# bghira/SimpleTuner

Hardware: NVIDIA H100
Metric: images/sec Flux.1-dev LoRA bf16 1024^2 (higher is better)
Workload: dtype bf16

## Files before the change

simpletuner_b200/csrc/api.cu:

```cuda
#include <cuda.h>
#include <cudaTypedefs.h>
#include <cuda_runtime.h>

#include <algorithm>
#include <atomic>
#include <cstdarg>
#include <cstdio>
#include <cmath>
#include <cstdlib>
#include <cstring>
#include <mutex>
#include <string>
#include <unordered_map>

#include <climits>
#include "../../include/stb200.h"
#include "attn_bwd.cuh"
#include "attn_fwd.cuh"
#include "optim.cuh"
#include "elementwise.cuh"
#include "gemm.cuh"
#include "lokr.cuh"
#include "vae.cuh"
#include "wgrad.cuh"

namespace {

thread_local std::string g_err;
std::atomic<long long> g_launches{0};

int fail(int code, const char* fmt, ...) {
  char buf[512];
  va_list ap;
  va_start(ap, fmt);
  vsnprintf(buf, sizeof buf, fmt, ap);
  va_end(ap);
  g_err = buf;
  return code;
}

#define STB_CUDA(expr)                                                                       \
  do {                                                                                       \
    cudaError_t e_ = (expr);                                                                 \
    if (e_ != cudaSuccess) return fail(STB_ERR_CUDA, "%s: %s", #expr, cudaGetErrorString(e_)); \
  } while (0)

#define STB_LAUNCH_CHECK(name)                                                                  \
  do {                                                                                          \
    cudaError_t e_ = cudaGetLastError();                                                        \
    if (e_ != cudaSuccess) return fail(STB_ERR_CUDA, "launch %s: %s", name, cudaGetErrorString(e_)); \
    g_launches.fetch_add(1, std::memory_order_relaxed);                                         \
  } while (0)

int num_sms() {
  static int n = [] {
    int dev = 0, v = 0;
    if (cudaGetDevice(&dev) != cudaSuccess) return 0;
    if (cudaDeviceGetAttribute(&v, cudaDevAttrMultiProcessorCount, dev) != cudaSuccess) return 0;
    return v;
  }();
  return n;
}

int check_device() {
  static int ok = [] {
    int dev = 0, major = 0;
    if (cudaGetDevice(&dev) != cudaSuccess) return 0;
    if (cudaDeviceGetAttribute(&major, cudaDevAttrComputeCapabilityMajor, dev) != cudaSuccess) return 0;
    int minor = 0;
    if (cudaDeviceGetAttribute(&minor, cudaDevAttrComputeCapabilityMinor, dev) != cudaSuccess) return 0;
    return major == 9 && minor == 0 ? 1 : 0;
  }();
  if (!ok) return fail(STB_ERR_UNSUPPORTED, "libstb200 needs an sm_90 (H100) device; there is no CPU or other-arch fallback");
  return 0;
}

PFN_cuTensorMapEncodeTiled_v12000 encode_fn() {
  static PFN_cuTensorMapEncodeTiled_v12000 fn = [] {
    void* p = nullptr;
    cudaDriverEntryPointQueryResult q;
    if (cudaGetDriverEntryPoint("cuTensorMapEncodeTiled", &p, cudaEnableDefault, &q) != cudaSuccess) p = nullptr;
    return reinterpret_cast<PFN_cuTensorMapEncodeTiled_v12000>(p);
  }();
  return fn;
}

struct MapKey {
  const void* ptr;
  int rank;
  unsigned long long dims[4];
  unsigned long long strides[3];
  unsigned box[4];
  bool operator==(const MapKey& o) const { return std::memcmp(this, &o, sizeof(MapKey)) == 0; }
};
struct MapKeyHash {
  size_t operator()(const MapKey& k) const {
    const unsigned char* p = reinterpret_cast<const unsigned char*>(&k);
    size_t h = 1469598103934665603ull;
    for (size_t i = 0; i < sizeof(MapKey); ++i) h = (h ^ p[i]) * 1099511628211ull;
    return h;
  }
};
std::mutex g_map_mu;
std::unordered_map<MapKey, CUtensorMap, MapKeyHash> g_maps;

int make_map_strided(CUtensorMap* out, const void* ptr, int rank, const unsigned long long* dims,
                     const unsigned long long* strides_bytes, const unsigned* box, const unsigned* estrides) {
  auto fn = encode_fn();
  if (!fn) return fail(STB_ERR_CUDA, "cuTensorMapEncodeTiled entry point not available");
  if (reinterpret_cast<uintptr_t>(ptr) & 15) return fail(STB_ERR_ARG, "tensor base pointer must be 16-byte aligned");
  for (int i = 0; i + 1 < rank; ++i)
    if (strides_bytes[i] & 15) return fail(STB_ERR_ARG, "tensor stride %d (%llu bytes) must be a multiple of 16 bytes", i, strides_bytes[i]);
  cuuint64_t gdim[4];
  cuuint64_t gstr[3];
  cuuint32_t bx[4], es[4];
  for (int i = 0; i < rank; ++i) gdim[i] = dims[i], bx[i] = box[i], es[i] = estrides[i];
  for (int i = 0; i + 1 < rank; ++i) gstr[i] = strides_bytes[i];
  CUresult r = fn(out, CU_TENSOR_MAP_DATA_TYPE_BFLOAT16, rank, const_cast<void*>(ptr), gdim, gstr, bx, es,
                  CU_TENSOR_MAP_INTERLEAVE_NONE, CU_TENSOR_MAP_SWIZZLE_128B, CU_TENSOR_MAP_L2_PROMOTION_L2_256B,
                  CU_TENSOR_MAP_FLOAT_OOB_FILL_NONE);
  if (r != CUDA_SUCCESS) return fail(STB_ERR_CUDA, "cuTensorMapEncodeTiled failed with CUresult %d", int(r));
  return 0;
}

int make_map(CUtensorMap* out, const void* ptr, int rank, const unsigned long long* dims,
             const unsigned long long* strides_bytes, const unsigned* box) {
  MapKey key;
  std::memset(&key, 0, sizeof key);
  key.ptr = ptr;
  key.rank = rank;
  for (int i = 0; i < rank; ++i) key.dims[i] = dims[i], key.box[i] = box[i];
  for (int i = 0; i + 1 < rank; ++i) key.strides[i] = strides_bytes[i];
  {
    std::lock_guard<std::mutex> lk(g_map_mu);
    auto it = g_maps.find(key);
    if (it != g_maps.end()) {
      *out = it->second;
      return 0;
    }
  }
  static const unsigned unit[4] = {1, 1, 1, 1};
  if (int r = make_map_strided(out, ptr, rank, dims, strides_bytes, box, unit)) return r;
  {
    std::lock_guard<std::mutex> lk(g_map_mu);
    if (g_maps.size() > 65536) g_maps.clear();
    g_maps.emplace(key, *out);
  }
  return 0;
}

int make_token_map(CUtensorMap* out, const void* ptr, int C, int S, int B, long long s_stride, long long b_stride,
                   unsigned rows) {
  const unsigned long long d[3] = {(unsigned long long)C, (unsigned long long)S, (unsigned long long)B};
  const unsigned long long sb[2] = {(unsigned long long)s_stride * 2ull,
                                    (unsigned long long)(B == 1 ? s_stride * (long long)S : b_stride) * 2ull};
  const unsigned bx[3] = {64, rows, 1};
  return make_map(out, ptr, 3, d, sb, bx);
}

int make_head_map(CUtensorMap* out, const void* ptr, int HD, int H, int S, int B, long long sb, long long ss,
                  long long sh, unsigned rows) {
  const unsigned long long d[4] = {(unsigned long long)HD, (unsigned long long)H, (unsigned long long)S, (unsigned long long)B};
  const unsigned long long s[3] = {(unsigned long long)sh * 2ull, (unsigned long long)ss * 2ull, (unsigned long long)sb * 2ull};
  const unsigned bx[4] = {64, 1, rows, 1};
  return make_map(out, ptr, 4, d, s, bx);
}

template <auto Kernel>
int set_smem(int bytes) {
  static std::atomic<bool> done{false};
  if (done.load(std::memory_order_acquire)) return 0;
  STB_CUDA(cudaFuncSetAttribute(Kernel, cudaFuncAttributeMaxDynamicSharedMemorySize, bytes));
  done.store(true, std::memory_order_release);
  return 0;
}

template <int BN, int EPI, bool CONV>
int launch_gemm_kernel(const stb::GemmMaps& maps, const stb::GemmParams& p, cudaStream_t st, const char* name) {
  using Cfg = stb::GemmCfg<BN>;
  if (int r = set_smem<stb::gemm_bf16_tn_kernel<BN, EPI, CONV>>(Cfg::SMEM_BYTES)) return r;
  const long long tiles = (long long)((p.rows_per_batch + Cfg::BM - 1) / Cfg::BM) * p.num_batches * ((p.N + BN - 1) / BN);
  const int grid = (int)std::min<long long>(tiles, num_sms());
  stb::gemm_bf16_tn_kernel<BN, EPI, CONV><<<grid, 384, Cfg::SMEM_BYTES, st>>>(maps, p);
  STB_LAUNCH_CHECK(name);
  return 0;
}

template <int BN>
int launch_gemm(const stb_gemm_args* a, cudaStream_t st) {
  stb::GemmMaps maps;
  std::memset(&maps, 0, sizeof maps);
  stb::GemmParams p;
  std::memset(&p, 0, sizeof p);
  for (int s = 0; s < a->nseg; ++s) {
    const stb_gemm_seg& g = a->seg[s];
    if (g.K <= 0 || (g.K & 7)) return fail(STB_ERR_ARG, "segment %d: K=%d must be a positive multiple of 8", s, g.K);
    if (int r = make_token_map(&maps.a[s], g.a, g.K, a->rows_per_batch, a->num_batches, g.a_row_stride, g.a_batch_stride,
                               stb::GemmCfg<BN>::BM))
      return r;
    if (g.w_kn) {
      unsigned long long wd[2] = {(unsigned long long)a->N, (unsigned long long)g.K};
      unsigned long long ws[1] = {(unsigned long long)g.w_row_stride * 2ull};
      unsigned wb[2] = {64, 64};
      if (int r = make_map(&maps.w[s], g.w, 2, wd, ws, wb)) return r;
    } else {
      unsigned long long wd[2] = {(unsigned long long)g.K, (unsigned long long)a->N};
      unsigned long long ws[1] = {(unsigned long long)g.w_row_stride * 2ull};
      unsigned wb[2] = {64, (unsigned)BN};
      if (int r = make_map(&maps.w[s], g.w, 2, wd, ws, wb)) return r;
    }
    p.w_kn[s] = g.w_kn ? 1 : 0;
    p.kblocks[s] = (g.K + 63) / 64;
  }
  p.rows_per_batch = a->rows_per_batch;
  p.num_batches = a->num_batches;
  p.N = a->N;
  p.nseg = a->nseg;
  p.nan_to_num = a->nan_to_num;
  p.D = static_cast<__nv_bfloat16*>(a->d);
  p.d_batch_stride = a->d_batch_stride;
  p.d_row_stride = a->d_row_stride;
  p.bias = static_cast<const __nv_bfloat16*>(a->bias);
  p.gate = static_cast<const __nv_bfloat16*>(a->gate);
  p.gate_batch_stride = a->gate_batch_stride;
  p.res = static_cast<const __nv_bfloat16*>(a->res);
  p.res_batch_stride = a->res_batch_stride;
  p.res_row_stride = a->res_row_stride;
  p.aux = static_cast<__nv_bfloat16*>(a->aux);
  p.aux_batch_stride = a->aux_batch_stride;
  p.aux_row_stride = a->aux_row_stride;
  switch (a->epi) {
    case stb::EPI_STORE: return launch_gemm_kernel<BN, stb::EPI_STORE, false>(maps, p, st, "gemm_bf16_tn");
    case stb::EPI_GELU: return launch_gemm_kernel<BN, stb::EPI_GELU, false>(maps, p, st, "gemm_bf16_tn");
    case stb::EPI_GATE_RES: return launch_gemm_kernel<BN, stb::EPI_GATE_RES, false>(maps, p, st, "gemm_bf16_tn");
    case stb::EPI_MUL_DGELU: return launch_gemm_kernel<BN, stb::EPI_MUL_DGELU, false>(maps, p, st, "gemm_bf16_tn");
    case stb::EPI_ADD_RES: return launch_gemm_kernel<BN, stb::EPI_ADD_RES, false>(maps, p, st, "gemm_bf16_tn");
    case stb::EPI_MUL: return launch_gemm_kernel<BN, stb::EPI_MUL, false>(maps, p, st, "gemm_bf16_tn");
    case stb::EPI_QUICK_GELU: return launch_gemm_kernel<BN, stb::EPI_QUICK_GELU, false>(maps, p, st, "gemm_bf16_tn");
  }
  return fail(STB_ERR_ARG, "unknown epilogue %d", a->epi);
}

bool aligned16(const void* p) { return (reinterpret_cast<uintptr_t>(p) & 15) == 0; }

}

template <int HD, bool BIAS>
static int launch_attn_fwd(const stb::AttnFwdMaps& maps, const stb::AttnFwdParams& p, dim3 grid, cudaStream_t st) {
  constexpr int SMEM = stb::AttnFwdCfg<HD>::SMEM_BYTES;
  if (int r = set_smem<stb::attn_fwd_kernel<HD, BIAS>>(SMEM)) return r;
  stb::attn_fwd_kernel<HD, BIAS><<<grid, 384, SMEM, st>>>(maps, p);
  STB_LAUNCH_CHECK(BIAS ? "attn_fwd_bias" : "attn_fwd");
  return 0;
}

template <int HD>
static int launch_attn_bwd(const stb_attn_bwd_args* a, const stb::AttnBwdMaps& maps, const stb::AttnBwdParams& p,
                           cudaStream_t st) {
  {
    const long long warps = (long long)a->B * a->Sq * a->H;
    stb::attn_bwd_delta_kernel<HD><<<(unsigned)((warps + 7) / 8), 256, 0, st>>>(
        static_cast<const __nv_bfloat16*>(a->o), a->o_b, a->o_s, a->o_h,
        static_cast<const __nv_bfloat16*>(a->d_o), a->do_b, a->do_s, a->do_h, a->delta, a->B, a->H, a->Sq);
    STB_LAUNCH_CHECK("attn_bwd_delta");
  }
  constexpr int SMEM1 = stb::AttnBwdCfg<HD>::DKDV_SMEM_BYTES, SMEM2 = stb::AttnBwdCfg<HD>::DQ_SMEM_BYTES;
  if (int r = set_smem<stb::attn_bwd_dkdv_kernel<HD>>(SMEM1)) return r;
  if (int r = set_smem<stb::attn_bwd_dq_kernel<HD>>(SMEM2)) return r;
  stb::attn_bwd_dkdv_kernel<HD><<<dim3((a->Sk + 63) / 64, a->H, a->B), 384, SMEM1, st>>>(maps, p);
  STB_LAUNCH_CHECK("attn_bwd_dkdv");
  stb::attn_bwd_dq_kernel<HD><<<dim3((a->Sq + 127) / 128, a->H, a->B), 384, SMEM2, st>>>(maps, p);
  STB_LAUNCH_CHECK("attn_bwd_dq");
  return 0;
}

template <int BN, int OUT>
static int launch_wgrad(const stb::WgradMaps& maps, stb::WgradParams p, cudaStream_t st) {
  constexpr int SMEM = stb::WgradCfg<BN, OUT>::SMEM_BYTES;
  if (int r = set_smem<stb::wgrad_kernel<BN, OUT>>(SMEM)) return r;
  p.col_tiles = (p.K + BN - 1) / BN;
  const int units = p.splits * ((p.N + 127) / 128) * p.col_tiles;
  const int grid = OUT == stb::WGRAD_OUT_BF16_NK ? std::min(units, num_sms()) : units;
  stb::wgrad_kernel<BN, OUT><<<grid, 384, SMEM, st>>>(maps, p);
  STB_LAUNCH_CHECK(OUT == stb::WGRAD_OUT_BF16_NK ? "wgrad_full" : "wgrad_tn");
  return 0;
}

extern "C" {

const char* stb_last_error(void) { return g_err.c_str(); }
int stb_version(void) { return 100; }
long long stb_launch_count(void) { return g_launches.load(); }
void stb_reset_launch_count(void) { g_launches.store(0); }

int stb_gemm_bf16(const stb_gemm_args* a, void* stream) {
  if (int r = check_device()) return r;
  if (!a || a->nseg < 1 || a->nseg > 3) return fail(STB_ERR_ARG, "nseg must be 1..3");
  if (a->num_batches < 1 || a->rows_per_batch < 1 || a->N < 1) return fail(STB_ERR_ARG, "empty problem");
  if (!aligned16(a->d) || (a->d_row_stride & 7) || (a->d_batch_stride & 7))
    return fail(STB_ERR_ARG, "D must be 16-byte aligned with strides multiple of 8 elements");
  if (a->bias && !aligned16(a->bias)) return fail(STB_ERR_ARG, "bias must be 16-byte aligned");
  if (a->epi == STB_EPI_GATE_RES && (!a->gate || !a->res)) return fail(STB_ERR_ARG, "GATE_RES needs gate and res");
  if (a->epi == STB_EPI_GATE_RES && (!aligned16(a->gate) || (a->gate_batch_stride & 7)))
    return fail(STB_ERR_ARG, "gate must be 16-byte aligned");
  if ((a->epi == STB_EPI_GATE_RES || a->epi == STB_EPI_ADD_RES) &&
      (!a->res || !aligned16(a->res) || (a->res_row_stride & 7) || (a->res_batch_stride & 7)))
    return fail(STB_ERR_ARG, "res must be given, 16-byte aligned, strides multiple of 8");
  if ((a->epi == STB_EPI_MUL_DGELU || a->epi == STB_EPI_MUL) && !a->aux) return fail(STB_ERR_ARG, "MUL_DGELU / MUL need aux");
  if (a->aux && (!aligned16(a->aux) || (a->aux_row_stride & 7) || (a->aux_batch_stride & 7)))
    return fail(STB_ERR_ARG, "aux must be 16-byte aligned, strides multiple of 8");
  if (a->epi < 0 || a->epi > 6) return fail(STB_ERR_ARG, "unknown epilogue %d", a->epi);
  cudaStream_t st = static_cast<cudaStream_t>(stream);
  if (a->tile_mt < 0 || a->tile_mt > 3) return fail(STB_ERR_ARG, "unsupported tile config MT=%d", a->tile_mt);
  int bn = a->tile_bn;
  if (bn == 0) {
    bn = a->N <= 64 ? 64 : (a->rows_per_batch <= 64 && a->N > 128 ? 256 : 128);
  }
  if (bn == 256) return launch_gemm<256>(a, st);
  if (bn == 128) return launch_gemm<128>(a, st);
  if (bn == 64) return launch_gemm<64>(a, st);
  return fail(STB_ERR_ARG, "unsupported tile config BN=%d", bn);
}

int stb_attn_fwd(const stb_attn_fwd_args* a, void* stream) {
  if (int r = check_device()) return r;
  if (!a || a->B < 1 || a->H < 1 || a->Sq < 1 || a->Sk < 1) return fail(STB_ERR_ARG, "empty attention problem");
  if (a->HD != 128 && a->HD != 64) return fail(STB_ERR_UNSUPPORTED, "head_dim %d not supported (64 or 128)", a->HD);
  if (!aligned16(a->o) || (a->o_s & 7) || (a->o_h & 7) || (a->o_b & 7)) return fail(STB_ERR_ARG, "O alignment");
  cudaStream_t st = static_cast<cudaStream_t>(stream);
  stb::AttnFwdMaps maps;
  auto mk = [&](CUtensorMap* m, const void* ptr, long long sb, long long ss, long long sh, int S) {
    return make_head_map(m, ptr, a->HD, a->H, S, a->B, sb, ss, sh, 128);
  };
  if (int r = mk(&maps.q, a->q, a->q_b, a->q_s, a->q_h, a->Sq)) return r;
  if (int r = mk(&maps.k, a->k, a->k_b, a->k_s, a->k_h, a->Sk)) return r;
  if (int r = mk(&maps.v, a->v, a->v_b, a->v_s, a->v_h, a->Sk)) return r;
  stb::AttnFwdParams p;
  p.B = a->B; p.H = a->H; p.Sq = a->Sq; p.Sk = a->Sk;
  p.scale = a->scale;
  p.O = static_cast<__nv_bfloat16*>(a->o);
  p.o_b = a->o_b; p.o_s = a->o_s; p.o_h = a->o_h;
  p.lse = a->lse;
  p.bias = static_cast<const __nv_bfloat16*>(a->bias);
  p.bias_h = a->bias_h; p.bias_q = a->bias_q;
  p.inv_scale = a->scale != 0.f ? 1.f / a->scale : 0.f;
  const dim3 grid((a->Sq + 127) / 128, a->H, a->B);
  if (a->bias) {
    if (a->scale == 0.f || a->bias_q < a->Sk) return fail(STB_ERR_ARG, "attn_fwd bias: scale must be non-zero and bias_q >= Sk");
    return a->HD == 128 ? launch_attn_fwd<128, true>(maps, p, grid, st) : launch_attn_fwd<64, true>(maps, p, grid, st);
  }
  return a->HD == 128 ? launch_attn_fwd<128, false>(maps, p, grid, st) : launch_attn_fwd<64, false>(maps, p, grid, st);
}

int stb_attn_bwd(const stb_attn_bwd_args* a, void* stream) {
  if (int r = check_device()) return r;
  if (!a || a->B < 1 || a->H < 1 || a->Sq < 1 || a->Sk < 1) return fail(STB_ERR_ARG, "empty attention problem");
  if (a->HD != 128 && a->HD != 64) return fail(STB_ERR_UNSUPPORTED, "head_dim %d not supported (64 or 128)", a->HD);
  if (!a->lse || !a->delta) return fail(STB_ERR_ARG, "attn_bwd needs lse and a delta scratch buffer");
  auto al = [&](const void* ptr, long long sb, long long ss, long long sh) {
    return aligned16(ptr) && !(sb & 7) && !(ss & 7) && !(sh & 7);
  };
  if (!al(a->dq, a->dq_b, a->dq_s, a->dq_h) || !al(a->dk, a->dk_b, a->dk_s, a->dk_h) ||
      !al(a->dv, a->dv_b, a->dv_s, a->dv_h))
    return fail(STB_ERR_ARG, "dq/dk/dv must be 16-byte aligned with strides multiple of 8 elements");
  cudaStream_t st = static_cast<cudaStream_t>(stream);
  stb::AttnBwdMaps maps;
  auto mk = [&](CUtensorMap* m, const void* ptr, long long sb, long long ss, long long sh, int S, unsigned rows) {
    return make_head_map(m, ptr, a->HD, a->H, S, a->B, sb, ss, sh, rows);
  };
  if (int r = mk(&maps.q128, a->q, a->q_b, a->q_s, a->q_h, a->Sq, 128)) return r;
  if (int r = mk(&maps.do128, a->d_o, a->do_b, a->do_s, a->do_h, a->Sq, 128)) return r;
  if (int r = mk(&maps.q64, a->q, a->q_b, a->q_s, a->q_h, a->Sq, 64)) return r;
  if (int r = mk(&maps.k64, a->k, a->k_b, a->k_s, a->k_h, a->Sk, 64)) return r;
  if (int r = mk(&maps.v64, a->v, a->v_b, a->v_s, a->v_h, a->Sk, 64)) return r;
  if (int r = mk(&maps.do64, a->d_o, a->do_b, a->do_s, a->do_h, a->Sq, 64)) return r;
  stb::AttnBwdParams p;
  p.B = a->B; p.H = a->H; p.Sq = a->Sq; p.Sk = a->Sk;
  p.scale = a->scale;
  p.lse = a->lse;
  p.delta = a->delta;
  p.dq = static_cast<__nv_bfloat16*>(a->dq);
  p.dk = static_cast<__nv_bfloat16*>(a->dk);
  p.dv = static_cast<__nv_bfloat16*>(a->dv);
  p.dq_b = a->dq_b; p.dq_s = a->dq_s; p.dq_h = a->dq_h;
  p.dk_b = a->dk_b; p.dk_s = a->dk_s; p.dk_h = a->dk_h;
  p.dv_b = a->dv_b; p.dv_s = a->dv_s; p.dv_h = a->dv_h;
  p.fuse_prep = 0;
  if (const stb_qk_prep* f = a->qk_prep) {
    if (a->Sq != a->Sk) return fail(STB_ERR_ARG, "qk_prep fusion needs self-attention (Sq == Sk)");
    if (!f->src || !aligned16(f->src) || (f->src_b & 7) || (f->src_s & 7) || (f->k_off & 7))
      return fail(STB_ERR_ARG, "qk_prep.src must be 16-byte aligned with strides / k_off multiple of 8 elements");
    if ((f->cos_t == nullptr) != (f->sin_t == nullptr)) return fail(STB_ERR_ARG, "qk_prep: give both cos_t and sin_t or neither");
    p.fuse_prep = 1;
    p.src = static_cast<const __nv_bfloat16*>(f->src);
    p.src_b = f->src_b; p.src_s = f->src_s; p.k_off = f->k_off;
    p.wq0 = static_cast<const __nv_bfloat16*>(f->wq); p.wk0 = static_cast<const __nv_bfloat16*>(f->wk);
    p.wq1 = static_cast<const __nv_bfloat16*>(f->wq_added); p.wk1 = static_cast<const __nv_bfloat16*>(f->wk_added);
    p.s_split = f->s_split;
    p.cosT = f->cos_t; p.sinT = f->sin_t;
    p.eps = f->eps;
  }
  p.q = static_cast<const __nv_bfloat16*>(a->q);
  p.d_o = static_cast<const __nv_bfloat16*>(a->d_o);
  p.q_b = a->q_b; p.q_s = a->q_s; p.q_h = a->q_h;
  p.do_b = a->do_b; p.do_s = a->do_s; p.do_h = a->do_h;
  if (a->HD == 128) return launch_attn_bwd<128>(a, maps, p, st);
  return launch_attn_bwd<64>(a, maps, p, st);
}

int stb_ln_modulate_fwd(const void* x, long long x_b, long long x_s, const void* shift, const void* scale,
                        long long mod_b, void* out, long long o_b, long long o_s, int B, int S, int D,
                        float eps, void* stream) {
  if (int r = check_device()) return r;
  if ((D & 7) || D > 8192) return fail(STB_ERR_ARG, "D=%d must be a multiple of 8 and <= 8192", D);
  if (!aligned16(x) || !aligned16(out) || !aligned16(shift) || !aligned16(scale) || (x_s & 7) || (x_b & 7) ||
      (o_s & 7) || (o_b & 7) || (mod_b & 7))
    return fail(STB_ERR_ARG, "ln_modulate_fwd alignment");
  cudaStream_t st = static_cast<cudaStream_t>(stream);
  const int rows = B * S;
  const int vpt = (D + 1023) / 1024;
  auto X = static_cast<const __nv_bfloat16*>(x);
  auto SH = static_cast<const __nv_bfloat16*>(shift);
  auto SC = static_cast<const __nv_bfloat16*>(scale);
  auto O = static_cast<__nv_bfloat16*>(out);
#define STB_LN_F(V) stb::ln_modulate_fwd_kernel<V><<<rows, 128, 0, st>>>(X, x_b, x_s, SH, SC, mod_b, O, o_b, o_s, S, D, eps)
  switch (vpt) {
    case 1: STB_LN_F(1); break;
    case 2: STB_LN_F(2); break;
    case 3: STB_LN_F(3); break;
    case 4: STB_LN_F(4); break;
    default: STB_LN_F(8); break;
  }
#undef STB_LN_F
  STB_LAUNCH_CHECK("ln_modulate_fwd");
  return 0;
}

int stb_ln_modulate_bwd(const void* dy, long long dy_b, long long dy_s, const void* x, long long x_b,
                        long long x_s, const void* scale, long long mod_b, const void* add, long long add_b,
                        long long add_s, void* dx, long long dx_b, long long dx_s, int B, int S, int D,
                        float eps, void* stream) {
  if (int r = check_device()) return r;
  if ((D & 7) || D > 4096) return fail(STB_ERR_ARG, "D=%d must be a multiple of 8 and <= 4096", D);
  if (!aligned16(x) || !aligned16(dy) || !aligned16(dx) || !aligned16(scale) || (add && !aligned16(add)))
    return fail(STB_ERR_ARG, "ln_modulate_bwd alignment");
  cudaStream_t st = static_cast<cudaStream_t>(stream);
  const int rows = B * S;
  const int vpt = (D + 1023) / 1024;
  auto DY = static_cast<const __nv_bfloat16*>(dy);
  auto X = static_cast<const __nv_bfloat16*>(x);
  auto SC = static_cast<const __nv_bfloat16*>(scale);
  auto AD = static_cast<const __nv_bfloat16*>(add);
  auto DX = static_cast<__nv_bfloat16*>(dx);
#define STB_LN_B(V) \
  stb::ln_modulate_bwd_kernel<V><<<rows, 128, 0, st>>>(DY, dy_b, dy_s, X, x_b, x_s, SC, mod_b, AD, add_b, add_s, DX, dx_b, dx_s, S, D, eps)
  switch (vpt) {
    case 1: STB_LN_B(1); break;
    case 2: STB_LN_B(2); break;
    case 3: STB_LN_B(3); break;
    default: STB_LN_B(4); break;
  }
#undef STB_LN_B
  STB_LAUNCH_CHECK("ln_modulate_bwd");
  return 0;
}

int stb_qk_rmsnorm_rope_fwd(const void* src, long long src_b, long long src_s, int k_off, const void* wq,
                            const void* wk, const void* wq_added, const void* wk_added, int s_split,
                            const float* cos_t, const float* sin_t, void* q_out, void* k_out,
                            long long dst_b, long long dst_s, int B, int S, int H, int HD, float eps,
                            void* stream) {
  if (int r = check_device()) return r;
  if (HD != 128 && HD != 64) return fail(STB_ERR_UNSUPPORTED, "head_dim %d not supported", HD);
// ... 517 lines not shown
```

simpletuner_b200/csrc/common.cuh:

```cuda
#pragma once
#include <cuda.h>
#include <cuda_bf16.h>
#include <cuda_runtime.h>
#include <stdint.h>

#include "wgmma.cuh"

#ifndef STB_WATCHDOG
#define STB_WATCHDOG 1
#endif

namespace stb {

__device__ __forceinline__ uint32_t smem_u32(const void* p) {
  return static_cast<uint32_t>(__cvta_generic_to_shared(p));
}
__device__ __forceinline__ uint32_t lane_id() { return threadIdx.x & 31u; }

__device__ __forceinline__ bool elect_one() {
  uint32_t pred = 0;
  asm volatile(
      "{\n\t"
      ".reg .pred P;\n\t"
      "elect.sync _|P, 0xffffffff;\n\t"
      "selp.u32 %0, 1, 0, P;\n\t"
      "}\n"
      : "=r"(pred));
  return pred != 0;
}

__device__ __forceinline__ void mbar_init(uint32_t bar, uint32_t count) {
  asm volatile("mbarrier.init.shared::cta.b64 [%0], %1;" ::"r"(bar), "r"(count) : "memory");
}
__device__ __forceinline__ void fence_mbar_init() {
  asm volatile("fence.mbarrier_init.release.cluster;" ::: "memory");
}
__device__ __forceinline__ void fence_proxy_async_smem() {
  asm volatile("fence.proxy.async.shared::cta;" ::: "memory");
}
__device__ __forceinline__ void mbar_arrive(uint32_t bar) {
  asm volatile("mbarrier.arrive.shared::cta.b64 _, [%0];" ::"r"(bar) : "memory");
}
__device__ __forceinline__ void mbar_arrive_expect_tx(uint32_t bar, uint32_t bytes) {
  asm volatile("mbarrier.arrive.expect_tx.shared::cta.b64 _, [%0], %1;" ::"r"(bar), "r"(bytes)
               : "memory");
}
__device__ __forceinline__ bool mbar_try_wait(uint32_t bar, uint32_t parity) {
  uint32_t ok;
  asm volatile(
      "{\n\t"
      ".reg .pred P;\n\t"
      "mbarrier.try_wait.parity.shared::cta.b64 P, [%1], %2;\n\t"
      "selp.u32 %0, 1, 0, P;\n\t"
      "}\n"
      : "=r"(ok)
      : "r"(bar), "r"(parity)
      : "memory");
  return ok != 0;
}

__device__ unsigned int g_stb_wedge[8];

__device__ __forceinline__ void mbar_wedged(uint32_t bar, uint32_t parity, int tag) {
  g_stb_wedge[0] = 0xdeadu;
  g_stb_wedge[1] = blockIdx.x;
  g_stb_wedge[2] = threadIdx.x;
  g_stb_wedge[3] = (unsigned)tag;
  g_stb_wedge[4] = bar;
  g_stb_wedge[5] = parity;
  __threadfence_system();
  __trap();
}

__device__ __forceinline__ void mbar_wait(uint32_t bar, uint32_t parity, int tag = 0) {
#if STB_WATCHDOG
  if (mbar_try_wait(bar, parity)) return;
  long long t0 = clock64();
  uint32_t spins = 0;
  while (!mbar_try_wait(bar, parity)) {
    if ((++spins & 0x3ffu) == 0 && (clock64() - t0) > 4000000000ll) mbar_wedged(bar, parity, tag);
  }
#else
  while (!mbar_try_wait(bar, parity)) {
  }
#endif
}

template <int STAGES>
struct StageRing {
  uint32_t bars;
  int stage = 0;
  uint32_t phase = 0;

  __device__ __forceinline__ uint32_t full_bar(int s) const { return bars + 8u * s; }
  __device__ __forceinline__ uint32_t empty_bar(int s) const { return bars + 8u * (STAGES + s); }
  __device__ __forceinline__ void init(uint32_t consumer_warps) const {
    for (int s = 0; s < STAGES; ++s) {
      mbar_init(full_bar(s), 1);
      mbar_init(empty_bar(s), consumer_warps);
    }
    fence_mbar_init();
  }
  __device__ __forceinline__ void advance() {
    if (++stage == STAGES) {
      stage = 0;
      phase ^= 1u;
    }
  }
  __device__ __forceinline__ void skip(int n) {
    stage += n;
    const int laps = stage / STAGES;
    stage -= laps * STAGES;
    phase ^= uint32_t(laps) & 1u;
  }
  __device__ __forceinline__ void wait_empty(int tag) const { mbar_wait(empty_bar(stage), phase ^ 1u, tag); }
  __device__ __forceinline__ void wait_full(int tag) const { mbar_wait(full_bar(stage), phase, tag); }
  __device__ __forceinline__ void release(int s) const {
    if (lane_id() == 0) mbar_arrive(empty_bar(s));
  }
};

__device__ __forceinline__ void tma_prefetch_desc(const CUtensorMap* m) {
  asm volatile("prefetch.tensormap [%0];" ::"l"(reinterpret_cast<uint64_t>(m)) : "memory");
}
__device__ __forceinline__ void tma_load_2d(uint32_t dst, const CUtensorMap* m, uint32_t bar, int c0,
                                            int c1) {
  asm volatile(
      "cp.async.bulk.tensor.2d.shared::cluster.global.mbarrier::complete_tx::bytes [%0], [%1, {%3, "
      "%4}], [%2];"
      ::"r"(dst), "l"(reinterpret_cast<uint64_t>(m)), "r"(bar), "r"(c0), "r"(c1)
      : "memory");
}
__device__ __forceinline__ void tma_load_3d(uint32_t dst, const CUtensorMap* m, uint32_t bar, int c0,
                                            int c1, int c2) {
  asm volatile(
      "cp.async.bulk.tensor.3d.shared::cluster.global.mbarrier::complete_tx::bytes [%0], [%1, {%3, "
      "%4, %5}], [%2];"
      ::"r"(dst), "l"(reinterpret_cast<uint64_t>(m)), "r"(bar), "r"(c0), "r"(c1), "r"(c2)
      : "memory");
}
__device__ __forceinline__ void tma_load_4d(uint32_t dst, const CUtensorMap* m, uint32_t bar, int c0,
                                            int c1, int c2, int c3) {
  asm volatile(
      "cp.async.bulk.tensor.4d.shared::cluster.global.mbarrier::complete_tx::bytes [%0], [%1, {%3, "
      "%4, %5, %6}], [%2];"
      ::"r"(dst), "l"(reinterpret_cast<uint64_t>(m)), "r"(bar), "r"(c0), "r"(c1), "r"(c2), "r"(c3)
      : "memory");
}
__device__ __forceinline__ void tma_store_4d(const CUtensorMap* m, uint32_t src, int c0, int c1, int c2,
                                             int c3) {
  asm volatile(
      "cp.async.bulk.tensor.4d.global.shared::cta.bulk_group [%0, {%2, %3, %4, %5}], [%1];"
      ::"l"(reinterpret_cast<uint64_t>(m)), "r"(src), "r"(c0), "r"(c1), "r"(c2), "r"(c3)
      : "memory");
}
__device__ __forceinline__ void tma_reduce_add_4d(const CUtensorMap* m, uint32_t src, int c0, int c1,
                                                  int c2, int c3) {
  asm volatile(
      "cp.reduce.async.bulk.tensor.4d.global.shared::cta.add.tile.bulk_group [%0, {%2, %3, %4, %5}], "
      "[%1];"
      ::"l"(reinterpret_cast<uint64_t>(m)), "r"(src), "r"(c0), "r"(c1), "r"(c2), "r"(c3)
      : "memory");
}
__device__ __forceinline__ void tma_store_commit() { asm volatile("cp.async.bulk.commit_group;" ::: "memory"); }
template <int N>
__device__ __forceinline__ void tma_store_wait_read() {
  asm volatile("cp.async.bulk.wait_group.read %0;" ::"n"(N) : "memory");
}
template <int N>
__device__ __forceinline__ void tma_store_wait() {
  asm volatile("cp.async.bulk.wait_group %0;" ::"n"(N) : "memory");
}

__device__ __forceinline__ void wg_fence() { asm volatile("wgmma.fence.sync.aligned;" ::: "memory"); }
__device__ __forceinline__ void wg_commit() { asm volatile("wgmma.commit_group.sync.aligned;" ::: "memory"); }
template <int N>
__device__ __forceinline__ void wg_wait() {
  asm volatile("wgmma.wait_group.sync.aligned %0;" ::"n"(N) : "memory");
}
template <int R>
__device__ __forceinline__ void wg_fence_regs(float (&d)[R]) {
#pragma unroll
  for (int i = 0; i < R; ++i) asm volatile("" : "+f"(d[i])::"memory");
}

__device__ __forceinline__ uint64_t sdesc_k(uint32_t tile_saddr, uint32_t byte_off) {
  const uint32_t lo = (tile_saddr >> 4) + (byte_off >> 4) + (1u << 16);
  const uint32_t hi = (1024u >> 4) | (1u << 30);
  return (uint64_t(hi) << 32) | lo;
}
__device__ __forceinline__ uint64_t sdesc_mn(uint32_t tile_saddr, uint32_t byte_off, uint32_t lbo) {
  const uint32_t lo = (tile_saddr >> 4) + ((byte_off >> 4) + ((lbo >> 4) << 16));
  const uint32_t hi = (1024u >> 4) | (1u << 30);
  return (uint64_t(hi) << 32) | lo;
}

template <int N>
__device__ __forceinline__ void reg_alloc() {
  asm volatile("setmaxnreg.inc.sync.aligned.u32 %0;" ::"n"(N));
}
template <int N>
__device__ __forceinline__ void reg_dealloc() {
  asm volatile("setmaxnreg.dec.sync.aligned.u32 %0;" ::"n"(N));
}

__device__ __forceinline__ uint32_t pack_bf16x2(float lo, float hi) {
  __nv_bfloat162 v = __floats2bfloat162_rn(lo, hi);
  return *reinterpret_cast<uint32_t*>(&v);
}
__device__ __forceinline__ float bf16_lo(uint32_t v) { return __uint_as_float(v << 16); }
__device__ __forceinline__ float bf16_hi(uint32_t v) { return __uint_as_float(v & 0xffff0000u); }
__device__ __forceinline__ float ex2f(float x) {
  float y;
  asm("ex2.approx.ftz.f32 %0, %1;" : "=f"(y) : "f"(x));
  return y;
}
__device__ __forceinline__ float gelu_tanh(float x) {
  const float k0 = 0.7978845608028654f, k1 = 0.044715f;
  float u = k0 * (x + k1 * x * x * x);
  return 0.5f * x * (1.f + tanhf(u));
}
__device__ __forceinline__ float gelu_tanh_grad(float x) {
  const float k0 = 0.7978845608028654f, k1 = 0.044715f;
  float x2 = x * x;
  float u = k0 * (x + k1 * x * x2);
  float t = tanhf(u);
  float du = k0 * (1.f + 3.f * k1 * x2);
  return 0.5f * (1.f + t) + 0.5f * x * (1.f - t * t) * du;
}

}
```

simpletuner_b200/csrc/gemm.cuh:

```cuda
#pragma once
#include <type_traits>
#include "common.cuh"

namespace stb {

enum GemmEpi : int {
  EPI_STORE = 0,
  EPI_GELU = 1,
  EPI_GATE_RES = 2,
  EPI_MUL_DGELU = 3,
  EPI_ADD_RES = 4,
  EPI_MUL = 5,
  EPI_QUICK_GELU = 6,
};

struct GemmParams {
  int rows_per_batch;
  int num_batches;
  int N;
  int nseg;
  int kblocks[3];
  int w_kn[3];
  int nan_to_num;
  __nv_bfloat16* D;
  long long d_batch_stride, d_row_stride;
  const __nv_bfloat16* bias;
  const __nv_bfloat16* gate;
  long long gate_batch_stride;
  const __nv_bfloat16* res;
  long long res_batch_stride, res_row_stride;
  __nv_bfloat16* aux;
  long long aux_batch_stride, aux_row_stride;
  int conv_h_out, conv_stride, conv_pad, conv_cblocks;
};

struct GemmMaps {
  CUtensorMap a[3];
  CUtensorMap w[3];
};

template <int BN>
struct GemmCfg {
  static constexpr int BM = BN == 256 ? 64 : 128;
  static constexpr int BK = 64;
  static constexpr int A_BYTES = BM * BK * 2;
  static constexpr int W_BYTES = BN * BK * 2;
  static constexpr int STAGE_BYTES = A_BYTES + W_BYTES;
  static constexpr int STAGES = (200 * 1024) / STAGE_BYTES > 8 ? 8 : (200 * 1024) / STAGE_BYTES;
  static constexpr int SMEM_BYTES = STAGES * STAGE_BYTES + 1024  + 256 ;
};

__device__ __forceinline__ float gemm_bf16r(float x) { return __bfloat162float(__float2bfloat16(x)); }

__device__ __forceinline__ void gemm_tile_coords(int tile, int tiles_m, int tiles_n, int& tm, int& tn) {
  constexpr int GM = 8;
  int per_group = GM * tiles_n;
  int g = tile / per_group;
  int first_m = g * GM;
  int gsize = min(GM, tiles_m - first_m);
  int within = tile - g * per_group;
  tm = first_m + within % gsize;
  tn = within / gsize;
}

__device__ __forceinline__ void ld_bf16x2(const __nv_bfloat16* p, bool two, float& a, float& b) {
  if (two) {
    const uint32_t u = *reinterpret_cast<const uint32_t*>(p);
    a = bf16_lo(u);
    b = bf16_hi(u);
  } else {
    a = __bfloat162float(p[0]);
    b = 0.f;
  }
}
__device__ __forceinline__ uint32_t ld_pair_word(const __nv_bfloat16* p, bool two) {
  return two ? *reinterpret_cast<const uint32_t*>(p) : uint32_t(__bfloat16_as_ushort(p[0]));
}
__device__ __forceinline__ void st_bf16x2(__nv_bfloat16* p, bool two, float a, float b) {
  if (two) *reinterpret_cast<uint32_t*>(p) = pack_bf16x2(a, b);
  else p[0] = __float2bfloat16(a);
}

template <int EPI>
constexpr bool kGemmEpiReadsRows = EPI == EPI_GATE_RES || EPI == EPI_ADD_RES || EPI == EPI_MUL_DGELU || EPI == EPI_MUL;
template <int EPI>
__device__ __forceinline__ const __nv_bfloat16* gemm_epi_row_operand(const GemmParams& p, int b, int s, int n) {
  if constexpr (EPI == EPI_GATE_RES || EPI == EPI_ADD_RES)
    return p.res + (long long)b * p.res_batch_stride + (long long)s * p.res_row_stride + n;
  else
    return p.aux + (long long)b * p.aux_batch_stride + (long long)s * p.aux_row_stride + n;
}

template <int EPI>
__device__ __forceinline__ void gemm_epi_pair(const GemmParams& p, int b, int s, int n, bool two, float f0, float f1,
                                              uint32_t x) {
  const long long drow = (long long)b * p.d_batch_stride + (long long)s * p.d_row_stride;
  __nv_bfloat16* xp = p.aux ? p.aux + (long long)b * p.aux_batch_stride + (long long)s * p.aux_row_stride + n : nullptr;
  if constexpr (EPI == EPI_GELU) {
    if (xp) st_bf16x2(xp, two, f0, f1);
    f0 = gelu_tanh(gemm_bf16r(f0));
    f1 = gelu_tanh(gemm_bf16r(f1));
  } else if constexpr (EPI == EPI_GATE_RES) {
    float g0, g1;
    ld_bf16x2(p.gate + (long long)b * p.gate_batch_stride + n, two, g0, g1);
    const float r0 = bf16_lo(x), r1 = bf16_hi(x);
    if (xp) st_bf16x2(xp, two, f0, f1);
    float o[2] = {r0 + gemm_bf16r(g0 * gemm_bf16r(f0)), r1 + gemm_bf16r(g1 * gemm_bf16r(f1))};
    if (p.nan_to_num) {
#pragma unroll
      for (int j = 0; j < 2; ++j) {
        float v = gemm_bf16r(o[j]);
        if (v != v) v = 0.f;
        else if (v == INFINITY) v = 65504.f;
        else if (v == -INFINITY) v = -65504.f;
        o[j] = v;
      }
    }
    f0 = o[0];
    f1 = o[1];
  } else if constexpr (EPI == EPI_MUL_DGELU) {
    f0 *= gelu_tanh_grad(bf16_lo(x));
    f1 *= gelu_tanh_grad(bf16_hi(x));
  } else if constexpr (EPI == EPI_MUL) {
    f0 = gemm_bf16r(f0) * bf16_lo(x);
    f1 = gemm_bf16r(f1) * bf16_hi(x);
  } else if constexpr (EPI == EPI_QUICK_GELU) {
    const float y0 = gemm_bf16r(f0), y1 = gemm_bf16r(f1);
    f0 = y0 / (1.f + __expf(-1.702f * y0));
    f1 = y1 / (1.f + __expf(-1.702f * y1));
  } else if constexpr (EPI == EPI_ADD_RES) {
    f0 += bf16_lo(x);
    f1 += bf16_hi(x);
  }
  st_bf16x2(p.D + drow + n, two, f0, f1);
}

template <int BN, int TB>
__device__ __forceinline__ void gemm_wgmma(float (&acc)[BN / 2], uint64_t a, uint64_t b, uint32_t accumulate) {
  if constexpr (BN == 256) wgmma_ss_n256<0, TB>(acc, a, b, accumulate);
  else if constexpr (BN == 128) wgmma_ss_n128<0, TB>(acc, a, b, accumulate);
  else wgmma_ss_n64<0, TB>(acc, a, b, accumulate);
}

template <int BN, int EPI, bool CONV = false>
__global__ void __launch_bounds__(384, 1)
gemm_bf16_tn_kernel(const __grid_constant__ GemmMaps maps, const GemmParams p) {
  using Cfg = GemmCfg<BN>;
  constexpr int STAGES = Cfg::STAGES;
  constexpr int MI = Cfg::BM / 64;

  extern __shared__ uint8_t smem_raw[];
  const uint32_t smem_base = (smem_u32(smem_raw) + 1023u) & ~1023u;
  StageRing<STAGES> ring{smem_base + STAGES * Cfg::STAGE_BYTES};
  const uint32_t order_bars = ring.bars + 16u * STAGES;

  const int warp = threadIdx.x >> 5;
  const int lane = threadIdx.x & 31;
  const int wg = __shfl_sync(0xffffffffu, warp >> 2, 0);

  const int tiles_per_batch = (p.rows_per_batch + Cfg::BM - 1) / Cfg::BM;
  const int tiles_m = tiles_per_batch * p.num_batches;
  const int tiles_n = (p.N + BN - 1) / BN;
  const int num_tiles = tiles_m * tiles_n;
  int nk = 0;
  for (int s = 0; s < p.nseg; ++s) nk += p.kblocks[s];

  if (threadIdx.x == 0) {
    for (int s = 0; s < p.nseg; ++s) {
      tma_prefetch_desc(&maps.a[s]);
      tma_prefetch_desc(&maps.w[s]);
    }
    ring.init(4);
    mbar_init(order_bars, 4);
    mbar_init(order_bars + 8, 4);
    fence_mbar_init();
  }
  __syncthreads();

  if (wg == 0) {
    reg_dealloc<40>();
    if (warp == 0) {
      for (int tile = blockIdx.x; tile < num_tiles; tile += gridDim.x) {
        int tm, tn;
        gemm_tile_coords(tile, tiles_m, tiles_n, tm, tn);
        const int b = tm / tiles_per_batch;
        const int s0 = (tm - b * tiles_per_batch) * Cfg::BM;
        const int n0 = tn * BN;
        for (int seg = 0; seg < p.nseg; ++seg) {
          for (int kb = 0; kb < p.kblocks[seg]; ++kb) {
            ring.wait_empty(1);
            const uint32_t sa = smem_base + ring.stage * Cfg::STAGE_BYTES;
            const uint32_t full = ring.full_bar(ring.stage);
            if (elect_one()) {
              mbar_arrive_expect_tx(full, Cfg::STAGE_BYTES);
              if constexpr (CONV) {
                const int tap = kb / p.conv_cblocks;
                const int c0 = (kb - tap * p.conv_cblocks) * 64;
                const int img = b / p.conv_h_out, yo = b - img * p.conv_h_out;
                const int dy = tap / 3, dx = tap - dy * 3;
                tma_load_4d(sa, &maps.a[0], full, c0, s0 * p.conv_stride + dx - p.conv_pad,
                            yo * p.conv_stride + dy - p.conv_pad, img);
              } else {
                tma_load_3d(sa, &maps.a[seg], full, kb * 64, s0, b);
              }
              if (p.w_kn[seg]) {
#pragma unroll
                for (int g = 0; g < BN / 64; ++g)
                  tma_load_2d(sa + Cfg::A_BYTES + g * 8192, &maps.w[seg], full, n0 + g * 64, kb * 64);
              } else {
                tma_load_2d(sa + Cfg::A_BYTES, &maps.w[seg], full, kb * 64, n0);
              }
            }
            __syncwarp();
            ring.advance();
          }
        }
      }
    }
  } else {
    reg_alloc<232>();
    const int cw = wg - 1;
    const int wq = warp & 3;
    uint32_t order_phase = 0;
    if (cw == 1) ring.skip(nk);
    float acc[MI][BN / 2];
    for (int tile = blockIdx.x + cw * gridDim.x; tile < num_tiles; tile += 2 * gridDim.x) {
      if (tile != (int)blockIdx.x) {
        mbar_wait(order_bars + 8u * cw, order_phase, 4);
        order_phase ^= 1u;
      }
      int tm, tn;
      gemm_tile_coords(tile, tiles_m, tiles_n, tm, tn);
      const int b = tm / tiles_per_batch;
      const int s0 = (tm - b * tiles_per_batch) * Cfg::BM;
      const int n0 = tn * BN;
      uint32_t accumulate = 0;
      int prev_stage = -1;
      for (int seg = 0; seg < p.nseg; ++seg) {
        const bool wkn = __shfl_sync(0xffffffffu, p.w_kn[seg], 0) != 0;
        for (int kb = 0; kb < p.kblocks[seg]; ++kb) {
          ring.wait_full(3);
          const uint32_t sa = smem_base + ring.stage * Cfg::STAGE_BYTES;
          const uint32_t sw = sa + Cfg::A_BYTES;
          wg_fence();
          if (wkn) {
#pragma unroll
            for (int kk = 0; kk < 4; ++kk)
#pragma unroll
              for (int mi = 0; mi < MI; ++mi)
                gemm_wgmma<BN, 1>(acc[mi], sdesc_k(sa + mi * 8192, kk * 32), sdesc_mn(sw, kk * 2048, 8192),
                                  kk > 0 ? 1u : accumulate);
          } else {
#pragma unroll
            for (int kk = 0; kk < 4; ++kk)
#pragma unroll
              for (int mi = 0; mi < MI; ++mi)
                gemm_wgmma<BN, 0>(acc[mi], sdesc_k(sa + mi * 8192, kk * 32), sdesc_k(sw, kk * 32),
                                  kk > 0 ? 1u : accumulate);
          }
          accumulate = 1;
          wg_commit();
          wg_wait<1>();
#pragma unroll
          for (int mi = 0; mi < MI; ++mi) wg_fence_regs(acc[mi]);
          if (prev_stage >= 0) ring.release(prev_stage);
          prev_stage = ring.stage;
          ring.advance();
        }
      }
      if (tile + (int)gridDim.x < num_tiles && lane == 0) mbar_arrive(order_bars + 8u * (cw ^ 1));
      ring.skip(nk);
      wg_wait<0>();
#pragma unroll
      for (int mi = 0; mi < MI; ++mi) wg_fence_regs(acc[mi]);
      ring.release(prev_stage);

      constexpr int CH = BN / 8 < 8 ? BN / 8 : 8;
      const bool b_ok = b < p.num_batches;
#pragma unroll
      for (int mi = 0; mi < MI; ++mi) {
        const int r_lo = s0 + mi * 64 + wq * 16 + (lane >> 2);
#pragma unroll
        for (int i0 = 0; i0 < BN / 8; i0 += CH) {
          uint32_t x[CH][2];
#pragma unroll
          for (int c = 0; c < CH; ++c) {
            const int n = n0 + 8 * (i0 + c) + 2 * (lane & 3);
#pragma unroll
            for (int h = 0; h < 2; ++h) {
              x[c][h] = 0;
              if constexpr (kGemmEpiReadsRows<EPI>)
                if (n < p.N && r_lo + 8 * h < p.rows_per_batch && b_ok)
                  x[c][h] = ld_pair_word(gemm_epi_row_operand<EPI>(p, b, r_lo + 8 * h, n), n + 1 < p.N);
            }
          }
#pragma unroll
          for (int c = 0; c < CH; ++c) {
            const int i = i0 + c;
            const int n = n0 + 8 * i + 2 * (lane & 3);
            if (n < p.N) {
              const bool two = n + 1 < p.N;
              float b0 = 0.f, b1 = 0.f;
              if (p.bias) ld_bf16x2(p.bias + n, two, b0, b1);
#pragma unroll
              for (int h = 0; h < 2; ++h) {
                const int s = r_lo + 8 * h;
                if (s < p.rows_per_batch && b_ok)
                  gemm_epi_pair<EPI>(p, b, s, n, two, acc[mi][4 * i + 2 * h] + b0, acc[mi][4 * i + 2 * h + 1] + b1,
                                     x[c][h]);
              }
            }
          }
        }
      }
    }
  }
}

}
```

Baseline: 1.864.

## Add 2-CTA cluster GEMM with multicast TMA weight loads for GELU epilogues

Adds a clustered variant of the bf16 TN GEMM in which two CTAs working on adjacent M tiles share the weight tile. Each CTA loads half of it and multicasts that half to both via TMA, and stage release is signalled to both CTAs' empty barriers. It is enabled by default for BN=128 GELU/MUL_DGELU GEMMs with at least 16 M tiles. The goal is to halve per-CTA weight traffic from L2. The cost is cross-CTA barrier coupling and fewer resident clusters. The wgmma commit/wait is also moved into each branch and the per-iteration register fences are dropped.

```diff
diff --git a/simpletuner_b200/csrc/api.cu b/simpletuner_b200/csrc/api.cu
--- a/simpletuner_b200/csrc/api.cu
+++ b/simpletuner_b200/csrc/api.cu
@@ -175,19 +175,46 @@
   return 0;
 }
 
-template <int BN, int EPI, bool CONV>
+template <int BN, int EPI, bool CONV, int CLUSTER = 1>
 int launch_gemm_kernel(const stb::GemmMaps& maps, const stb::GemmParams& p, cudaStream_t st, const char* name) {
   using Cfg = stb::GemmCfg<BN>;
-  if (int r = set_smem<stb::gemm_bf16_tn_kernel<BN, EPI, CONV>>(Cfg::SMEM_BYTES)) return r;
-  const long long tiles = (long long)((p.rows_per_batch + Cfg::BM - 1) / Cfg::BM) * p.num_batches * ((p.N + BN - 1) / BN);
-  const int grid = (int)std::min<long long>(tiles, num_sms());
-  stb::gemm_bf16_tn_kernel<BN, EPI, CONV><<<grid, 384, Cfg::SMEM_BYTES, st>>>(maps, p);
+  constexpr auto kernel = stb::gemm_bf16_tn_kernel<BN, EPI, CONV, CLUSTER>;
+  if (int r = set_smem<kernel>(Cfg::SMEM_BYTES)) return r;
+  const long long tiles_m = (long long)((p.rows_per_batch + Cfg::BM - 1) / Cfg::BM) * p.num_batches;
+  const long long units = (tiles_m + CLUSTER - 1) / CLUSTER * ((p.N + BN - 1) / BN);
+  if constexpr (CLUSTER == 1) {
+    const int grid = (int)std::min<long long>(units, num_sms());
+    kernel<<<grid, 384, Cfg::SMEM_BYTES, st>>>(maps, p);
+  } else {
+    cudaLaunchConfig_t cfg;
+    std::memset(&cfg, 0, sizeof cfg);
+    cudaLaunchAttribute attr[1];
+    attr[0].id = cudaLaunchAttributeClusterDimension;
+    attr[0].val.clusterDim.x = CLUSTER;
+    attr[0].val.clusterDim.y = 1;
+    attr[0].val.clusterDim.z = 1;
+    cfg.blockDim = dim3(384);
+    cfg.dynamicSmemBytes = Cfg::SMEM_BYTES;
+    cfg.stream = st;
+    cfg.attrs = attr;
+    cfg.numAttrs = 1;
+    static std::atomic<int> max_clusters{0};
+    int mc = max_clusters.load(std::memory_order_acquire);
+    if (mc == 0) {
+      cfg.gridDim = dim3(CLUSTER * (num_sms() / CLUSTER));
+      STB_CUDA(cudaOccupancyMaxActiveClusters(&mc, kernel, &cfg));
+      if (mc < 1) return fail(STB_ERR_CUDA, "%s: no %d-CTA cluster of this kernel fits on the device", name, CLUSTER);
+      max_clusters.store(mc, std::memory_order_release);
+    }
+    cfg.gridDim = dim3((unsigned)(CLUSTER * std::min<long long>(units, mc)));
+    STB_CUDA(cudaLaunchKernelEx(&cfg, kernel, maps, p));
+  }
   STB_LAUNCH_CHECK(name);
   return 0;
 }
 
 template <int BN>
-int launch_gemm(const stb_gemm_args* a, cudaStream_t st) {
+int launch_gemm(const stb_gemm_args* a, cudaStream_t st, bool cluster) {
   stb::GemmMaps maps;
   std::memset(&maps, 0, sizeof maps);
   stb::GemmParams p;
@@ -206,7 +233,7 @@
     } else {
       unsigned long long wd[2] = {(unsigned long long)g.K, (unsigned long long)a->N};
       unsigned long long ws[1] = {(unsigned long long)g.w_row_stride * 2ull};
-      unsigned wb[2] = {64, (unsigned)BN};
+      unsigned wb[2] = {64, cluster ? 64u : (unsigned)BN};
       if (int r = make_map(&maps.w[s], g.w, 2, wd, ws, wb)) return r;
     }
     p.w_kn[s] = g.w_kn ? 1 : 0;
@@ -229,14 +256,20 @@
   p.aux = static_cast<__nv_bfloat16*>(a->aux);
   p.aux_batch_stride = a->aux_batch_stride;
   p.aux_row_stride = a->aux_row_stride;
+  auto go = [&](auto epi) -> int {
+    constexpr int EPI = decltype(epi)::value;
+    if constexpr (BN == 128)
+      if (cluster) return launch_gemm_kernel<BN, EPI, false, 2>(maps, p, st, "gemm_bf16_tn_cluster");
+    return launch_gemm_kernel<BN, EPI, false>(maps, p, st, "gemm_bf16_tn");
+  };
   switch (a->epi) {
-    case stb::EPI_STORE: return launch_gemm_kernel<BN, stb::EPI_STORE, false>(maps, p, st, "gemm_bf16_tn");
-    case stb::EPI_GELU: return launch_gemm_kernel<BN, stb::EPI_GELU, false>(maps, p, st, "gemm_bf16_tn");
-    case stb::EPI_GATE_RES: return launch_gemm_kernel<BN, stb::EPI_GATE_RES, false>(maps, p, st, "gemm_bf16_tn");
-    case stb::EPI_MUL_DGELU: return launch_gemm_kernel<BN, stb::EPI_MUL_DGELU, false>(maps, p, st, "gemm_bf16_tn");
-    case stb::EPI_ADD_RES: return launch_gemm_kernel<BN, stb::EPI_ADD_RES, false>(maps, p, st, "gemm_bf16_tn");
-    case stb::EPI_MUL: return launch_gemm_kernel<BN, stb::EPI_MUL, false>(maps, p, st, "gemm_bf16_tn");
-    case stb::EPI_QUICK_GELU: return launch_gemm_kernel<BN, stb::EPI_QUICK_GELU, false>(maps, p, st, "gemm_bf16_tn");
+    case stb::EPI_STORE: return go(std::integral_constant<int, stb::EPI_STORE>{});
+    case stb::EPI_GELU: return go(std::integral_constant<int, stb::EPI_GELU>{});
+    case stb::EPI_GATE_RES: return go(std::integral_constant<int, stb::EPI_GATE_RES>{});
+    case stb::EPI_MUL_DGELU: return go(std::integral_constant<int, stb::EPI_MUL_DGELU>{});
+    case stb::EPI_ADD_RES: return go(std::integral_constant<int, stb::EPI_ADD_RES>{});
+    case stb::EPI_MUL: return go(std::integral_constant<int, stb::EPI_MUL>{});
+    case stb::EPI_QUICK_GELU: return go(std::integral_constant<int, stb::EPI_QUICK_GELU>{});
   }
   return fail(STB_ERR_ARG, "unknown epilogue %d", a->epi);
 }
@@ -311,14 +344,19 @@
     return fail(STB_ERR_ARG, "aux must be 16-byte aligned, strides multiple of 8");
   if (a->epi < 0 || a->epi > 6) return fail(STB_ERR_ARG, "unknown epilogue %d", a->epi);
   cudaStream_t st = static_cast<cudaStream_t>(stream);
-  if (a->tile_mt < 0 || a->tile_mt > 3) return fail(STB_ERR_ARG, "unsupported tile config MT=%d", a->tile_mt);
+  if (a->tile_mt < 0 || a->tile_mt > 2) return fail(STB_ERR_ARG, "unsupported tile config MT=%d", a->tile_mt);
   int bn = a->tile_bn;
   if (bn == 0) {
     bn = a->N <= 64 ? 64 : (a->rows_per_batch <= 64 && a->N > 128 ? 256 : 128);
   }
-  if (bn == 256) return launch_gemm<256>(a, st);
-  if (bn == 128) return launch_gemm<128>(a, st);
-  if (bn == 64) return launch_gemm<64>(a, st);
+  if (bn == 256) return launch_gemm<256>(a, st, false);
+  if (bn == 128) {
+    const long long tiles_m = (long long)((a->rows_per_batch + 127) / 128) * a->num_batches;
+    const bool cluster = a->tile_mt == 2 || (a->tile_mt == 0 && tiles_m >= 16 &&
+                                             (a->epi == STB_EPI_GELU || a->epi == STB_EPI_MUL_DGELU));
+    return launch_gemm<128>(a, st, cluster);
+  }
+  if (bn == 64) return launch_gemm<64>(a, st, false);
   return fail(STB_ERR_ARG, "unsupported tile config BN=%d", bn);
 }
 
diff --git a/simpletuner_b200/csrc/common.cuh b/simpletuner_b200/csrc/common.cuh
--- a/simpletuner_b200/csrc/common.cuh
+++ b/simpletuner_b200/csrc/common.cuh
@@ -57,6 +57,24 @@
       : "r"(bar), "r"(parity)
       : "memory");
   return ok != 0;
+}
+
+__device__ __forceinline__ uint32_t cluster_ctarank() {
+  uint32_t r;
+  asm volatile("mov.u32 %0, %%cluster_ctarank;" : "=r"(r));
+  return r;
+}
+__device__ __forceinline__ void cluster_sync() {
+  asm volatile("barrier.cluster.arrive.release.aligned;\n\tbarrier.cluster.wait.acquire.aligned;" ::: "memory");
+}
+__device__ __forceinline__ void mbar_arrive_remote(uint32_t bar, uint32_t rank) {
+  asm volatile(
+      "{\n\t"
+      ".reg .b32 ra;\n\t"
+      "mapa.shared::cluster.u32 ra, %0, %1;\n\t"
+      "mbarrier.arrive.shared::cluster.b64 _, [ra];\n\t"
+      "}\n" ::"r"(bar), "r"(rank)
+      : "memory");
 }
 
 __device__ unsigned int g_stb_wedge[8];
@@ -118,6 +136,12 @@
   __device__ __forceinline__ void release(int s) const {
     if (lane_id() == 0) mbar_arrive(empty_bar(s));
   }
+  __device__ __forceinline__ void release_cluster(int s, uint32_t peer) const {
+    if (lane_id() == 0) {
+      mbar_arrive(empty_bar(s));
+      mbar_arrive_remote(empty_bar(s), peer);
+    }
+  }
 };
 
 __device__ __forceinline__ void tma_prefetch_desc(const CUtensorMap* m) {
@@ -129,6 +153,14 @@
       "cp.async.bulk.tensor.2d.shared::cluster.global.mbarrier::complete_tx::bytes [%0], [%1, {%3, "
       "%4}], [%2];"
       ::"r"(dst), "l"(reinterpret_cast<uint64_t>(m)), "r"(bar), "r"(c0), "r"(c1)
+      : "memory");
+}
+__device__ __forceinline__ void tma_load_2d_mc(uint32_t dst, const CUtensorMap* m, uint32_t bar, int c0, int c1,
+                                               uint16_t cta_mask) {
+  asm volatile(
+      "cp.async.bulk.tensor.2d.shared::cluster.global.mbarrier::complete_tx::bytes.multicast::cluster [%0], [%1, "
+      "{%3, %4}], [%2], %5;"
+      ::"r"(dst), "l"(reinterpret_cast<uint64_t>(m)), "r"(bar), "r"(c0), "r"(c1), "h"(cta_mask)
       : "memory");
 }
 __device__ __forceinline__ void tma_load_3d(uint32_t dst, const CUtensorMap* m, uint32_t bar, int c0,
@@ -185,12 +217,12 @@
 }
 
 __device__ __forceinline__ uint64_t sdesc_k(uint32_t tile_saddr, uint32_t byte_off) {
-  const uint32_t lo = (tile_saddr >> 4) + (byte_off >> 4) + (1u << 16);
+  const uint32_t lo = ((tile_saddr & 0x3ffffu) >> 4) + (byte_off >> 4) + (1u << 16);
   const uint32_t hi = (1024u >> 4) | (1u << 30);
   return (uint64_t(hi) << 32) | lo;
 }
 __device__ __forceinline__ uint64_t sdesc_mn(uint32_t tile_saddr, uint32_t byte_off, uint32_t lbo) {
-  const uint32_t lo = (tile_saddr >> 4) + ((byte_off >> 4) + ((lbo >> 4) << 16));
+  const uint32_t lo = ((tile_saddr & 0x3ffffu) >> 4) + ((byte_off >> 4) + ((lbo >> 4) << 16));
   const uint32_t hi = (1024u >> 4) | (1u << 30);
   return (uint64_t(hi) << 32) | lo;
 }
diff --git a/simpletuner_b200/csrc/gemm.cuh b/simpletuner_b200/csrc/gemm.cuh
--- a/simpletuner_b200/csrc/gemm.cuh
+++ b/simpletuner_b200/csrc/gemm.cuh
@@ -142,12 +142,13 @@
   else wgmma_ss_n64<0, TB>(acc, a, b, accumulate);
 }
 
-template <int BN, int EPI, bool CONV = false>
+template <int BN, int EPI, bool CONV = false, int CLUSTER = 1>
 __global__ void __launch_bounds__(384, 1)
 gemm_bf16_tn_kernel(const __grid_constant__ GemmMaps maps, const GemmParams p) {
   using Cfg = GemmCfg<BN>;
   constexpr int STAGES = Cfg::STAGES;
   constexpr int MI = Cfg::BM / 64;
+  static_assert(CLUSTER == 1 || (CLUSTER == 2 && BN == 128 && !CONV), "2-CTA clusters: 128 x 128 GEMM tiles only");
 
   extern __shared__ uint8_t smem_raw[];
   const uint32_t smem_base = (smem_u32(smem_raw) + 1023u) & ~1023u;
@@ -161,7 +162,11 @@
   const int tiles_per_batch = (p.rows_per_batch + Cfg::BM - 1) / Cfg::BM;
   const int tiles_m = tiles_per_batch * p.num_batches;
   const int tiles_n = (p.N + BN - 1) / BN;
-  const int num_tiles = tiles_m * tiles_n;
+  const int units_m = (tiles_m + CLUSTER - 1) / CLUSTER;
+  const int num_units = units_m * tiles_n;
+  const int unit0 = blockIdx.x / CLUSTER;
+  const int units_stride = gridDim.x / CLUSTER;
+  const uint32_t rank = CLUSTER == 2 ? cluster_ctarank() : 0u;
   int nk = 0;
   for (int s = 0; s < p.nseg; ++s) nk += p.kblocks[s];
 
@@ -170,19 +175,21 @@
       tma_prefetch_desc(&maps.a[s]);
       tma_prefetch_desc(&maps.w[s]);
     }
-    ring.init(4);
+    ring.init(4 * CLUSTER);
     mbar_init(order_bars, 4);
     mbar_init(order_bars + 8, 4);
     fence_mbar_init();
   }
-  __syncthreads();
+  if constexpr (CLUSTER == 2) cluster_sync();
+  else __syncthreads();
 
   if (wg == 0) {
     reg_dealloc<40>();
     if (warp == 0) {
-      for (int tile = blockIdx.x; tile < num_tiles; tile += gridDim.x) {
+      for (int unit = unit0; unit < num_units; unit += units_stride) {
         int tm, tn;
-        gemm_tile_coords(tile, tiles_m, tiles_n, tm, tn);
+        gemm_tile_coords(unit, units_m, tiles_n, tm, tn);
+        tm = tm * CLUSTER + (int)rank;
         const int b = tm / tiles_per_batch;
         const int s0 = (tm - b * tiles_per_batch) * Cfg::BM;
         const int n0 = tn * BN;
@@ -203,7 +210,12 @@
               } else {
                 tma_load_3d(sa, &maps.a[seg], full, kb * 64, s0, b);
               }
-              if (p.w_kn[seg]) {
+              if constexpr (CLUSTER == 2) {
+                const int hn = n0 + 64 * (int)rank;
+                const uint32_t hw = sa + Cfg::A_BYTES + rank * 8192u;
+                if (p.w_kn[seg]) tma_load_2d_mc(hw, &maps.w[seg], full, hn, kb * 64, 0x3);
+                else tma_load_2d_mc(hw, &maps.w[seg], full, kb * 64, hn, 0x3);
+              } else if (p.w_kn[seg]) {
 #pragma unroll
                 for (int g = 0; g < BN / 64; ++g)
                   tma_load_2d(sa + Cfg::A_BYTES + g * 8192, &maps.w[seg], full, n0 + g * 64, kb * 64);
@@ -224,13 +236,14 @@
     uint32_t order_phase = 0;
     if (cw == 1) ring.skip(nk);
     float acc[MI][BN / 2];
-    for (int tile = blockIdx.x + cw * gridDim.x; tile < num_tiles; tile += 2 * gridDim.x) {
-      if (tile != (int)blockIdx.x) {
+    for (int unit = unit0 + cw * units_stride; unit < num_units; unit += 2 * units_stride) {
+      if (unit != unit0) {
         mbar_wait(order_bars + 8u * cw, order_phase, 4);
         order_phase ^= 1u;
       }
       int tm, tn;
-      gemm_tile_coords(tile, tiles_m, tiles_n, tm, tn);
+      gemm_tile_coords(unit, units_m, tiles_n, tm, tn);
+      tm = tm * CLUSTER + (int)rank;
       const int b = tm / tiles_per_batch;
       const int s0 = (tm - b * tiles_per_batch) * Cfg::BM;
       const int n0 = tn * BN;
@@ -250,6 +263,8 @@
               for (int mi = 0; mi < MI; ++mi)
                 gemm_wgmma<BN, 1>(acc[mi], sdesc_k(sa + mi * 8192, kk * 32), sdesc_mn(sw, kk * 2048, 8192),
                                   kk > 0 ? 1u : accumulate);
+            wg_commit();
+            wg_wait<1>();
           } else {
 #pragma unroll
             for (int kk = 0; kk < 4; ++kk)
@@ -257,23 +272,25 @@
               for (int mi = 0; mi < MI; ++mi)
                 gemm_wgmma<BN, 0>(acc[mi], sdesc_k(sa + mi * 8192, kk * 32), sdesc_k(sw, kk * 32),
                                   kk > 0 ? 1u : accumulate);
+            wg_commit();
+            wg_wait<1>();
           }
           accumulate = 1;
-          wg_commit();
-          wg_wait<1>();
-#pragma unroll
-          for (int mi = 0; mi < MI; ++mi) wg_fence_regs(acc[mi]);
-          if (prev_stage >= 0) ring.release(prev_stage);
+          if (prev_stage >= 0) {
+            if constexpr (CLUSTER == 2) ring.release_cluster(prev_stage, rank ^ 1u);
+            else ring.release(prev_stage);
+          }
           prev_stage = ring.stage;
           ring.advance();
         }
       }
-      if (tile + (int)gridDim.x < num_tiles && lane == 0) mbar_arrive(order_bars + 8u * (cw ^ 1));
+      if (unit + units_stride < num_units && lane == 0) mbar_arrive(order_bars + 8u * (cw ^ 1));
       ring.skip(nk);
       wg_wait<0>();
 #pragma unroll
       for (int mi = 0; mi < MI; ++mi) wg_fence_regs(acc[mi]);
-      ring.release(prev_stage);
+      if constexpr (CLUSTER == 2) ring.release_cluster(prev_stage, rank ^ 1u);
+      else ring.release(prev_stage);
 
       constexpr int CH = BN / 8 < 8 ? BN / 8 : 8;
       const bool b_ok = b < p.num_batches;
@@ -315,6 +332,7 @@
       }
     }
   }
-}
-
-}
+  if constexpr (CLUSTER == 2) cluster_sync();
+}
+
+}
```

New measurement: 1.941 (median of 6 runs). +4.1%, better.
